# rmcar17/SpectralClusterSupertree

Measured on AMD Instinct MI355X. Metric: top-level PCG build + Fiedler solve wall-time (s) at N taxa, 1/2/4/8 MI355X, lower is better.
Workload: dtype f64 (loop operator: fp32 image of W; fp64 renewal + confirmation)

## Files before the change

include/scs_hip.h:

```cpp
#ifndef SCS_HIP_H
#define SCS_HIP_H

#include <stddef.h>
#include <stdint.h>

#ifdef __cplusplus
extern "C" {
#endif

#define SCS_OK 0
#define SCS_EINVAL (-1)
#define SCS_EHIP (-2)
#define SCS_ENOMEM (-3)
#define SCS_ECOMM (-4)
#define SCS_ENOCONV (-5)
#define SCS_EUNSUP (-6)

#define SCS_UNIQUE_ID_BYTES 128

typedef struct scs_ctx scs_ctx;
typedef struct scs_tables scs_tables;
typedef struct scs_graph scs_graph;

typedef struct scs_stats {
// ... 279 lines not shown
int scs_debug_update(scs_ctx *ctx, double *y, int32_t ldy, int32_t y_col0, int32_t kc, double alpha,
                     const double *a, int32_t lda, int32_t a_col0, int32_t ka, const double *c,
                     int32_t ldc, double sign, int32_t n);

int scs_debug_small_svqb(scs_ctx *ctx, const double *g, int32_t k, double drop_tol, double *t_out,
                         int32_t *mask_out);

int scs_debug_small_rr(scs_ctx *ctx, const double *tm, int32_t nparts, int32_t nq, int32_t b, const int32_t *mask,
                       double drop_tol, int32_t exact_from, int32_t start, double *c_out, double *d_out,
                       double *theta_out, int32_t *mask_p_out, int32_t *mask_out);

int scs_debug_small_orth(scs_ctx *ctx, const double *partial, int32_t nparts, int32_t b, double drop_tol,
                         const double *theta, int32_t layout, double *coef_out, int32_t *mask_out,
                         double *report_out);

#define SCS_DEBUG_PANEL_PAD 16
int scs_debug_panel(scs_ctx *ctx, int32_t which, int32_t b, int32_t n, const double *q, const double *aq,
                    const double *u, const double *coef_a, const double *coef_b, const double *theta,
                    const double *dinv, const double *ypart, int32_t nseg, int32_t blocks, double *q_out,
                    double *aq_out, double *partial_out, double *zt_out);

int scs_debug_comm_selftest(scs_ctx *ctx, int32_t count, const double *host_in, double *host_out);

int scs_debug_copy_bandwidth(scs_ctx *ctx, int64_t bytes, int32_t reps, double *gbs_out);

int scs_debug_scan(scs_ctx *ctx, int32_t op, int32_t n_parts, int64_t n, const int32_t *in, int32_t *out);

int scs_debug_graph_raw(scs_ctx *ctx, scs_graph *graph, int32_t what, void *out, int32_t *info_out);

int scs_debug_block_records(scs_ctx *ctx, const scs_tables *tables, int32_t t_begin, int32_t t_end, int32_t row_begin,
                            int32_t row_end, int32_t kind, int32_t *spos_out, double *gap_out, int32_t *argpos_out,
                            int32_t *depth_out, int32_t *cnt_out);

int scs_debug_split_plan(int32_t n_trees, const int64_t *node_off, int32_t *tpb_out, int32_t *n_groups_out,
                         uint8_t *staged_out);

int scs_debug_score_plan(const scs_tables *sources, int32_t n_trees, const int64_t *tree_off, int32_t super_leaves,
                         int32_t max_batch_trees, int64_t extra_per_leaf, int64_t extra_per_tree,
                         int32_t *n_batches_out, int32_t *bstart_out, int64_t *info_out, int32_t *words_out,
                         int32_t *zb_out, int64_t *wg_out);

int scs_debug_branch_plan(const scs_tables *sources, int32_t n_trees, const int64_t *tree_off, int32_t super_leaves,
                          int32_t max_batch_trees, int64_t extra_per_leaf, int64_t extra_per_tree,
                          int32_t max_lds_bytes, int32_t *n_batches_out, int32_t *bstart_out, int64_t *bt_out,
                          int64_t *tx_out, int64_t *call_out);

int scs_debug_placement_plan(const scs_tables *sources, int32_t n_trees, const int64_t *tree_off, int32_t super_leaves,
                             int32_t max_batch_trees, int32_t max_lds_bytes, int32_t n_queries,
                             int32_t n_sub_queries, int32_t n_degrees, const int32_t *degrees, int32_t *n_batches_out,
                             int32_t *bstart_out, int64_t *pl_out, int64_t *cp_out, int64_t *blk_out, int64_t *py_out);

int scs_debug_parsimony_plan(const scs_tables *sources, int32_t n_trees, const int64_t *tree_off, const int64_t *chars,
                             int32_t n_nodes, const int32_t *parent, int32_t max_batch_trees, int32_t max_pass_words,
                             int32_t *n_batches_out, int32_t *bstart_out, int64_t *info_out, int64_t *batch_out);

int scs_debug_source_pairs_plan(const scs_tables *sources, int32_t n_trees, const int64_t *tree_off, int32_t n_taxa,
                                int32_t n_rows, int32_t max_batch_trees, int32_t max_lds_bytes, int32_t *n_batches_out,
                                int32_t *bstart_out, int64_t *info_out, int64_t *tile_out);

int scs_debug_coverage_plan(const scs_tables *sources, int32_t n_trees, const int64_t *tree_off, int32_t n_taxa,
                            int32_t n_rows, int32_t min_trees, int32_t max_batch_rows, int32_t max_reg_words,
                            int32_t matrices_wanted, int64_t *info_out, int64_t *batches_out);

#ifdef __cplusplus
}
#endif
// ... 2 lines not shown
```

spectralclustersupertree_amd/_native.py:

```python

from __future__ import annotations

import ctypes as C
from pathlib import Path

import numpy as np

_PKG = Path(__file__).resolve().parent
LIB_PATH = _PKG / "libscs_hip.so"

UNIQUE_ID_BYTES = 128
BUILD_MONOTONE = 1
BUILD_SHARED = 2
BUILD_UPPER = 4
BUILD_SCATTER = 8


class ScsError(RuntimeError):

    def __init__(self, code: int, message: str) -> None:
        super().__init__(f"libscs_hip error {code}: {message}")
        self.code = code


# ... 145 lines not shown
    "scs_graph_download": (C.c_int, [_P, _P, _DP]),
    "scs_graph_download_rows": (C.c_int, [_P, _P, _I32, _I32, _DP]),
    "scs_graph_degrees": (C.c_int, [_P, _P, _DP]),
    "scs_graph_free": (C.c_int, [_P, _P]),
    "scs_fiedler": (C.c_int, [_P, _P, _DP, C.c_double, _I32, _I32, _DP, C.POINTER(Stats)]),
    "scs_small_solve": (C.c_int, [_P, _I32, _IP, _IP, _IP, _IP, _IP, _IP, _DP, _DP, _IP, _DP, _DP, _DP]),
    "scs_small_solve_begin": (C.c_int, [_P, _I32, _IP, _IP, _IP, _IP, _IP, _IP, _DP, _DP, _IP, _I32,
                                        C.POINTER(C.c_int32)]),
    "scs_small_solve_begin_forest": (C.c_int, [_P, _P, _IP, _I32, _I32, _IP, _I32, _P]),
    "scs_small_solve_end": (C.c_int, [_P, _I32, _DP, _DP, _DP]),
    "scs_debug_small_inputs": (C.c_int, [_P, _I32, _IP, _IP, _IP, _DP, _DP]),
    "scs_debug_tables_download": (C.c_int, [_P, _P, _LP, _IP, _IP, _DP, _DP, _LP]),
    "scs_debug_loop_policy": (C.c_int, [C.c_double, _I32, C.c_double, C.c_double, _I32, _I32, _DP, _IP]),
    "scs_debug_jacobi": (C.c_int, [_P, _DP, _I32, _DP, _DP]),
    "scs_debug_gram": (C.c_int, [_P, _DP, _DP, _I32, _I32, _I32, _I32, _DP]),
    "scs_debug_apply": (C.c_int, [_P, _P, _DP, _I32, _DP]),
    "scs_debug_apply_ex": (C.c_int, [_P, _P, _DP, _I32, _I32, _I32, _DP, _IP]),
    "scs_debug_team_apply": (C.c_int, [_P, _P, _DP, _DP, _I32, _I32, _I32, _I32, _DP, _DP, _DP, _LP]),
    "scs_debug_gram_ex": (C.c_int, [_P, _DP, _I32, _I32, _I32, _DP, _I32, _I32, _I32, _I32, _I32, _I32, _DP]),
    "scs_debug_update": (C.c_int, [_P, _DP, _I32, _I32, _I32, C.c_double, _DP, _I32, _I32, _I32, _DP, _I32,
                                   C.c_double, _I32]),
    "scs_debug_small_svqb": (C.c_int, [_P, _DP, _I32, C.c_double, _DP, _IP]),
    "scs_debug_small_rr": (C.c_int, [_P, _DP, _I32, _I32, _I32, _IP, C.c_double, _I32, _I32, _DP, _DP, _DP, _IP,
                                     _IP]),
    "scs_debug_small_orth": (C.c_int, [_P, _DP, _I32, _I32, C.c_double, _DP, _I32, _DP, _IP, _DP]),
    "scs_debug_panel": (C.c_int, [_P, _I32, _I32, _I32, _DP, _DP, _DP, _DP, _DP, _DP, _DP, _DP, _I32, _I32, _DP,
                                  _DP, _DP, _DP]),
    "scs_debug_comm_selftest": (C.c_int, [_P, _I32, _DP, _DP]),
    "scs_debug_copy_bandwidth": (C.c_int, [_P, C.c_int64, _I32, _DP]),
    "scs_debug_scan": (C.c_int, [_P, _I32, _I32, C.c_int64, _IP, _IP]),
    "scs_debug_split_plan": (C.c_int, [_I32, _LP, _P, _P, _P]),
    "scs_debug_graph_raw": (C.c_int, [_P, _P, _I32, _P, _IP]),
    "scs_debug_block_records": (C.c_int, [_P, _P, _I32, _I32, _I32, _I32, _I32, _IP, _DP, _IP, _IP, _IP]),
    "scs_debug_score_plan": (C.c_int, [_P, _I32, _LP, _I32, _I32, C.c_int64, C.c_int64, _P, _IP, _LP, _IP, _IP, _LP]),
    "scs_debug_branch_plan": (C.c_int, [_P, _I32, _LP, _I32, _I32, C.c_int64, C.c_int64, _I32, _P, _IP, _LP, _LP, _LP]),
    "scs_debug_placement_plan": (C.c_int, [_P, _I32, _LP, _I32, _I32, _I32, _I32, _I32, _I32, _IP, _IP, _IP, _LP, _LP,
                                           _LP, _LP]),
    "scs_debug_parsimony_plan": (C.c_int, [_P, _I32, _LP, _LP, _I32, _IP, _I32, _I32, _P, _IP, _LP, _LP]),
    "scs_debug_source_pairs_plan": (C.c_int, [_P, _I32, _LP, _I32, _I32, _I32, _I32, _P, _IP, _LP, _LP]),
    "scs_debug_coverage_plan": (C.c_int, [_P, _I32, _LP, _I32, _I32, _I32, _I32, _I32, _I32, _LP, _LP]),
}

_lib = None


def load_library() -> C.CDLL:
    global _lib
    if _lib is not None:
        return _lib
    if not LIB_PATH.exists():
        msg = (
            f"{LIB_PATH} not found: build it with `python -c 'import __graft_entry__ as g; g.build()'` "
            "or `make -C spectralclustersupertree_amd/csrc`.  There is no CPU fallback."
        )
        raise ImportError(msg)
    lib = C.CDLL(str(LIB_PATH))
    for name, (restype, argtypes) in SIGNATURES.items():
        fn = getattr(lib, name)
        fn.restype = restype
        fn.argtypes = argtypes
    have = int(lib.scs_version())
    if have != ABI_VERSION:
        msg = f"{LIB_PATH} reports ABI version {have}, this package binds {ABI_VERSION}: rebuild the library"
        raise ImportError(msg)
    _lib = lib
    return lib
# ... 48 lines not shown
```

spectralclustersupertree_amd/backend.py:

```python

from __future__ import annotations

import ctypes as C
import os

import numpy as np

from spectralclustersupertree_amd import _env
from spectralclustersupertree_amd import _native as nv
from spectralclustersupertree_amd.flatten import TreeTables

DEFAULT_TOL = 1e-13
DEFAULT_MAX_ITER = 2000

_M, _N, _Q, _QN, _QK = ("m",), ("n_nodes",), ("nq",), ("nq", "n_nodes"), ("nq", "top_k")


def _resident_solve() -> bool:
    return bool(int(_env.probe("SCS_RESIDENT_SOLVE", "1")))


class Device:

    def __init__(self, device: int = 0, rank: int = 0, world: int = 1, unique_id: bytes | None = None,
# ... 684 lines not shown
    out["py_bstart"] = bstart[2, : k + 1].astype(np.int64)
    rows = py.reshape(-1)[: k * len(deg) * 4].reshape(k, len(deg), 4)
    for i, key in enumerate(("words", "stride", "acc_lds", "lds")):
        out[f"py_{key}"] = rows[:, :, i].copy()
    return out


def debug_parsimony_plan(sources, parent, chars=None, batch_trees: int = 0, pass_words: int = 0) -> dict:
    handle, off = (sources._h, None) if isinstance(sources, DeviceTables) else (None, sources)
    if off is not None:
        off = np.ascontiguousarray(off, dtype=np.int64)
    m = sources.n_trees if off is None else len(off) - 1
    parent = np.ascontiguousarray(parent, dtype=np.int32)
    if chars is not None:
        chars = np.ascontiguousarray(chars, dtype=np.int64)
        if chars.shape != (m,):
            msg = f"chars must have one entry per source tree ({m}), not shape {chars.shape}"
            raise ValueError(msg)
    nb = C.c_int32(0)
    bstart = np.zeros(m + 1, dtype=np.int32)
    info = np.zeros(8, dtype=np.int64)
    rows = np.zeros((max(m, 1), 2), dtype=np.int64)
    nv.check(nv.load_library().scs_debug_parsimony_plan(
        handle, m, None if off is None else nv.lptr(off), None if chars is None else nv.lptr(chars), len(parent),
        nv.iptr(parent), int(batch_trees), int(pass_words), C.byref(nb), nv.iptr(bstart), nv.lptr(info),
        nv.lptr(rows)))
    k = int(nb.value)
    keys = ("pass_words", "frame_depth", "counter_bits", "lds_bytes", "frames_in_block", "extra_per_leaf",
            "extra_per_tree", "super_tips")
    return {"bstart": bstart[: k + 1].astype(np.int64), "passes": rows[:k, 0].copy(), "words": rows[:k, 1].copy(),
            **{key: int(info[i]) for i, key in enumerate(keys)}}


def debug_source_pairs_plan(sources, n_taxa: int = 0, n_rows: int | None = None, batch_trees: int = 0,
                            lds_bytes: int = 0) -> dict:
    handle, off = (sources._h, None) if isinstance(sources, DeviceTables) else (None, sources)
    if off is not None:
        off = np.ascontiguousarray(off, dtype=np.int64)
    m = sources.n_trees if off is None else len(off) - 1
    lib = nv.load_library()
    nb = C.c_int32(0)
    bstart = np.zeros(m + 1, dtype=np.int32)
    info = np.zeros(6, dtype=np.int64)
    args = (handle, m, None if off is None else nv.lptr(off), int(n_taxa), m if n_rows is None else int(n_rows),
            int(batch_trees), int(lds_bytes), C.byref(nb), nv.iptr(bstart), nv.lptr(info))
    nv.check(lib.scs_debug_source_pairs_plan(*args, None))
    k = int(nb.value)
    tiles = np.zeros((k, k, 7), dtype=np.int64)
    nv.check(lib.scs_debug_source_pairs_plan(*args, nv.lptr(tiles)))
    keys = ("levels", "row_stride", "slab_stride", "slab_wgs", "workspace", "lds_cap")
    return {"bstart": bstart[: k + 1].astype(np.int64), **{key: int(info[i]) for i, key in enumerate(keys)},
            "width": tiles[:, :, 0].copy(), "lds": tiles[:, :, 1].copy(), "slab": tiles[:, :, 2].copy(),
            "need": tiles[:, :, 3].copy(), "threads": tiles[:, :, 4].copy(), "grid_limit": tiles[:, :, 5].copy(),
            "rows_per_launch": tiles[:, :, 6].copy()}


def debug_coverage_plan(sources, n_taxa: int = 0, n_rows: int | None = None, min_trees: int = 1, batch_rows: int = 0,
                        reg_words: int = 0, matrices: int = 0) -> dict:
    handle, m = (sources._h, sources.n_trees) if isinstance(sources, DeviceTables) else (None, int(sources))
    lib = nv.load_library()
    info = np.zeros(12, dtype=np.int64)
    args = (handle, m, None, int(n_taxa), -1 if n_rows is None else int(n_rows), int(min_trees), int(batch_rows),
            int(reg_words), int(matrices), nv.lptr(info))
    nv.check(lib.scs_debug_coverage_plan(*args, None))
    batches = np.zeros((int(info[7]), 4), dtype=np.int64)
    nv.check(lib.scs_debug_coverage_plan(*args, nv.lptr(batches) if len(batches) else None))
# ... 151 lines not shown
        flags = nv.BUILD_MONOTONE if self.monotone else 0
        if upper:
            flags |= nv.BUILD_UPPER
            shared = False
        if scatter:
            flags |= nv.BUILD_SCATTER
            shared = False
        if shared is None:
            shared = self.dev.world > 1
        if shared:
            flags |= nv.BUILD_SHARED
        nv.check(self.dev._lib.scs_pcg_build(self.dev._ctx, self._h, row_begin, row_end, flags,
                                             C.byref(handle), C.byref(stats)))
        graph = DeviceGraph(self.dev, handle, stats.as_dict())
        graph.upper = bool(upper)
        return graph

    def block_records(self, kind: str, t_begin: int = 0, t_end: int | None = None, row_begin: int = 0,
                      row_end: int | None = None) -> dict:
        t_end = self.n_trees if t_end is None else t_end
        row_end = self.n_taxa if row_end is None else row_end
        code = {"mono": 0, "wide": 1, "general": 2}[kind]
        nb, nt = (max(row_end - row_begin, 0) + 63) // 64, max(t_end - t_begin, 0)
        spos = np.empty((nb, nt, 64), dtype=np.int32)
        gap = np.empty((nb, nt, 64), dtype=np.float64)
        argpos = np.empty((nb, nt, 64), dtype=np.int32)
        depth = np.empty((nb, nt, 64), dtype=np.int32) if code == 2 else None
        cnt = np.empty((nb, nt), dtype=np.int32)
        nv.check(self.dev._lib.scs_debug_block_records(
            self.dev._ctx, self._h, int(t_begin), int(t_end), int(row_begin), int(row_end), code, nv.iptr(spos),
            nv.dptr(gap), nv.iptr(argpos), nv.iptr(depth) if depth is not None else None, nv.iptr(cnt)))
        return {"spos": spos, "gap": gap, "argpos": argpos, "depth": depth, "cnt": cnt}


    def matrix_free_graph(self, max_block: int = 8) -> "DeviceGraph":
        handle = C.c_void_p()
        nv.check(self.dev._lib.scs_graph_matrix_free(self.dev._ctx, self._h, int(max_block), C.byref(handle)))
        return DeviceGraph(self.dev, handle, {})


class DeviceGraph:
    def __init__(self, dev: Device, handle, build_stats: dict | None = None) -> None:
        self.dev, self._h = dev, handle
        self.build_stats = build_stats or {}
        self.upper = False

    def free(self) -> None:
        if self._h:
            self.dev._lib.scs_graph_free(self.dev._ctx, self._h)
            self._h = C.c_void_p()

    def __del__(self) -> None:
        try:
            self.free()
        except Exception:
            pass

    @property
    def shape(self) -> tuple[int, int, int]:
        n, rb, re_ = C.c_int32(), C.c_int32(), C.c_int32()
        nv.check(self.dev._lib.scs_graph_shape(self._h, C.byref(n), C.byref(rb), C.byref(re_)))
        return n.value, rb.value, re_.value

    def contract(self, group_start: np.ndarray) -> "DeviceGraph":
        gs = np.ascontiguousarray(group_start, dtype=np.int32)
        handle = C.c_void_p()
# ... 109 lines not shown
```

spectralclustersupertree_amd/csrc/scs_build.hip:

```cpp

#include <algorithm>

#include "scs_internal.h"

typedef unsigned long long u64;
typedef unsigned int u32;

constexpr u32 DEPTH_INF = 0xFFFFFFFFu;


__device__ __forceinline__ void rmq_offsets(int m, int a, int b, int (&o)[2]) {
    const int k = 31 - __clz(b - a);
    o[0] = k * m + a;
    o[1] = k * m + b - (1 << k);
}

template <typename K>
__device__ __forceinline__ K rmq_min(const K *__restrict__ base, int m, int a, int b) {
    int o[2];
    rmq_offsets(m, a, b, o);
    const K x = base[o[0]], y = base[o[1]];
    return x < y ? x : y;
}

// ... 86 lines not shown
        const int half = 1 << (k - 1), last = m - (1 << k);
        const argmin_t *am_prev = am + (int64_t)(k - 2) * m;
        argmin_t *am_cur = am + (int64_t)(k - 1) * m;
        for (int p0 = threadIdx.x; p0 <= last; p0 += 1024 * FUSED_UNROLL) {
            K a[FUSED_UNROLL], b[FUSED_UNROLL];
            int oa[FUSED_UNROLL], ob[FUSED_UNROLL];
#pragma unroll
            for (int u = 0; u < FUSED_UNROLL; ++u) {
                const int p = p0 + u * 1024;
                oa[u] = ob[u] = 0;
                if (p <= last) {
                    a[u] = prev[p];
                    b[u] = prev[p + half];
                    if (k > 1) {
                        oa[u] = (int)am_prev[p];
                        ob[u] = (int)am_prev[p + half];
                    }
                }
            }
#pragma unroll
            for (int u = 0; u < FUSED_UNROLL; ++u) {
                const int p = p0 + u * 1024;
                if (p <= last) {
                    cur[p] = pick(a[u], b[u]);
                    am_cur[p] = (argmin_t)(pick.right_less(a[u], b[u]) ? half + ob[u] : oa[u]);
                }
            }
        }
        __syncthreads();
    }
}
constexpr int SPARSE_FUSED_MAX_LEAVES = 32768;
static_assert(SPARSE_FUSED_MAX_LEAVES <= (1 << ARGMIN_MAX_LEVEL), "every level of a fused table has an argmin level");
struct pick_smaller_value {
    __device__ double operator()(double a, double b) const { return a < b ? a : b; }
    __device__ bool right_less(double a, double b) const { return b < a; }
};

__device__ __forceinline__ double min_f64(double a, double b) {
#ifdef SCS_MIN_ASM
    double r;
    asm("v_min_f64 %0, %1, %2" : "=v"(r) : "v"(a), "v"(b));
    return r;
#else
    return __builtin_fmin(a, b);
#endif
}

#include "scs_mono.h"
#include "scs_mono_wide.h"
#include "scs_gen.h"
struct pick_shallower_pair {
    __device__ gap_entry operator()(const gap_entry a, const gap_entry b) const { return gap_min(a, b); }
    __device__ bool right_less(const gap_entry a, const gap_entry b) const { return b.d < a.d; }
};

__global__ __launch_bounds__(256) void k_scatter_atomic(const int64_t *__restrict__ tree_off,
                                                         const int32_t *__restrict__ leaf_taxon, int t0,
                                                         const int64_t *__restrict__ st_off,
                                                         const double *__restrict__ stv,
                                                         double *__restrict__ w, int64_t ld) {
    const int tl = blockIdx.y;
    const int64_t off = tree_off[t0 + tl];
    const int nl = (int)(tree_off[t0 + tl + 1] - off);
    const int m = nl - 1;
    const int nbk = (nl + 63) / 64;
// ... 387 lines not shown
__global__ void k_tile_lists(const int2 *__restrict__ tiles, int n_tiles, const unsigned char *__restrict__ rec,
                             int rec_bytes, int cnt_off, int n_batch, const unsigned char *__restrict__ pcol,
                             int32_t *__restrict__ lists, int32_t *__restrict__ list_cnt) {
    const int i = blockIdx.x * blockDim.x + threadIdx.x;
    if (i >= n_tiles) return;
    const int2 tile = tiles[i];
    const unsigned char *rb = rec + (int64_t)tile.x * n_batch * rec_bytes + cnt_off;
    const unsigned char *pc = pcol + (int64_t)tile.y * n_batch;
    int32_t *out = lists + (int64_t)i * n_batch;
    int c = 0;
    for (int t = 0; t < n_batch; ++t)
        if (pc[t] && *(const int *)(rb + (int64_t)t * rec_bytes) > 0) out[c++] = t;
    list_cnt[i] = c;
}

constexpr int PIPE_NG = 2;

namespace {

enum { PREP_MONO = 0, PREP_WIDE = 1, PREP_GEN = 2, PREP_NO_RECORDS = 3 };

struct prep_batch {
    const scs_tables *tb;
    int t0, nb;
    int kind;
    int32_t *pos;
    int64_t npad;
    const int64_t *st_off;
    const int64_t *am_off;
    void *st;
    argmin_t *am;
    unsigned char *rec;
    int n_blocks, row_begin, row_end;
};

int64_t table_entries(int64_t m) { return (int64_t)levels_for(m) * m; }
int64_t argmin_entries(int64_t m) { return (int64_t)argmin_levels(levels_for(m)) * m; }

int prep_piece(const prep_batch &b, int tl0, int np, hipStream_t s) {
    if (np <= 0) return SCS_OK;
    const scs_tables *tb = b.tb;
    int max_levels = 0;
    int64_t max_n = 0;
    for (int t = b.t0 + tl0; t < b.t0 + tl0 + np; ++t) {
        const int64_t nt = tb->h_tree_off[t + 1] - tb->h_tree_off[t];
        max_levels = std::max(max_levels, levels_for(nt - 1));
        max_n = std::max(max_n, nt);
    }
    const dim3 grid_l((unsigned)((max_n + 255) / 256), (unsigned)np);
    const dim3 grid_r((unsigned)b.n_blocks, (unsigned)np);
    const bool fused = max_n <= SPARSE_FUSED_MAX_LEAVES && max_levels > 1;
    if (b.kind != PREP_GEN) {
        double *st = (double *)b.st;
        k_positions_values<<<grid_l, 256, 0, s>>>(tb->d_tree_off, tb->d_leaf_taxon, tb->d_adj_depth, tb->d_adj_val,
                                                  tb->d_tree_w, b.t0, tl0, b.pos, b.npad, b.st_off, st);
        if (fused)
            k_sparse_levels_fused<double><<<(unsigned)np, 1024, 0, s>>>(tb->d_tree_off, b.t0, tl0, b.st_off, st, b.am_off,
                                                                        b.am, pick_smaller_value{});
        else
            for (int k = 1; k < max_levels; ++k)
                k_sparse_level<double><<<grid_l, 256, 0, s>>>(tb->d_tree_off, b.t0, tl0, k, b.st_off, st, b.am_off, b.am,
                                                              pick_smaller_value{});
        if (b.kind == PREP_WIDE)
            k_block_records_wide<PIPE_NG><<<grid_r, 64, 0, s>>>(tb->d_tree_off, b.t0, tl0, b.nb, b.pos, b.npad, b.st_off, st,
                                                          b.am_off, b.am, b.row_begin, b.row_end, b.rec);
        else if (b.kind == PREP_MONO)
            k_block_records_mono<<<grid_r, 64, 0, s>>>(tb->d_tree_off, b.t0, tl0, b.nb, b.pos, b.npad, b.st_off, st,
                                                       b.am_off, b.am, b.row_begin, b.row_end, b.rec);
    } else {
        gap_entry *st = (gap_entry *)b.st;
        k_positions_pairs<<<grid_l, 256, 0, s>>>(tb->d_tree_off, tb->d_leaf_taxon, tb->d_adj_depth, tb->d_adj_val,
                                                 tb->d_tree_w, b.t0, tl0, b.pos, b.npad, b.st_off, st);
        if (fused)
            k_sparse_levels_fused<gap_entry><<<(unsigned)np, 1024, 0, s>>>(tb->d_tree_off, b.t0, tl0, b.st_off, st,
                                                                           b.am_off, b.am, pick_shallower_pair{});
        else
            for (int k = 1; k < max_levels; ++k)
                k_sparse_level<gap_entry><<<grid_l, 256, 0, s>>>(tb->d_tree_off, b.t0, tl0, k, b.st_off, st, b.am_off,
                                                                 b.am, pick_shallower_pair{});
        k_block_records_gen<<<grid_r, 64, 0, s>>>(tb->d_tree_off, b.t0, tl0, b.nb, b.pos, b.npad, b.st_off, st, b.am_off,
                                                  b.am, b.row_begin, b.row_end, b.rec);
    }
    SCS_HIP_CHECK(hipGetLastError());
    return SCS_OK;
}

struct pinned_ref {
    scs_ctx *ctx;
    hipStream_t stream;
    void *p = nullptr;
    bool in_flight = false;
    pinned_ref(scs_ctx *c, hipStream_t s) : ctx(c), stream(s) {}
    ~pinned_ref() {
        if (!p) return;
        if (in_flight) hipStreamSynchronize(stream);
        scs_pinned_release(ctx, p);
    }
};

}

extern "C" int scs_pcg_build(scs_ctx *ctx, const scs_tables *tb, int32_t row_begin,
                             int32_t row_end, int32_t flags, scs_graph **out,
                             scs_build_stats *stats) {
    SCS_REQUIRE(ctx && tb && out, "scs_pcg_build: null argument");
    SCS_REQUIRE((flags & ~(SCS_BUILD_MONOTONE | SCS_BUILD_SHARED | SCS_BUILD_UPPER | SCS_BUILD_SCATTER)) == 0,
// ... 250 lines not shown
        const size_t need_pos = (size_t)nb * npad * 4;
        const size_t need_st = (size_t)h_st_off[nb] * entry_bytes + 64;
        const size_t need_am = (size_t)h_am_off[nb] * sizeof(argmin_t) + 64;
        const size_t need_rec = (size_t)n_blocks * nb * rec_bytes;
        const int wide_min_trees = wide_forced ? 1 : 96;
        const bool wide_b = wide && (nb >= wide_min_trees || (groups.size() >= 8 * 256 && nb >= 16));
        if (wide_b) {
            ++spec_batches;
            spec_trees += nb;
            single_batch_spec = true;
        }
        SCS_TRY(d_pos.alloc(need_pos));
        SCS_TRY(d_st.alloc(need_st));
        SCS_TRY(d_am.alloc(need_am));
        SCS_TRY(d_rec.alloc(need_rec));

        SCS_HIP_CHECK(hipEventRecord(ev_prep.a, s));
        SCS_HIP_CHECK(hipMemsetAsync(d_pos.p, 0xFF, need_pos, s));
        prep_batch pb;
        pb.tb = tb;
        pb.t0 = t0;
        pb.nb = nb;
        pb.kind = !monotone ? PREP_GEN : wide_b ? PREP_WIDE : scatter ? PREP_NO_RECORDS : PREP_MONO;
        pb.pos = (int32_t *)d_pos.p;
        pb.npad = npad;
        pb.st_off = (const int64_t *)d_stoff.p + off_at[bi];
        pb.am_off = pb.st_off + nb + 1;
        pb.st = d_st.p;
        pb.am = (argmin_t *)d_am.p;
        pb.rec = (unsigned char *)d_rec.p;
        pb.n_blocks = n_blocks;
        pb.row_begin = b_row_begin;
        pb.row_end = b_row_end;
        for (int p0 = t0; p0 < t1;) {
            int p1 = t1;
            if (by_arrival)
                for (const int32_t c : tb->late_start)
                    if (c > p0 && c < p1) p1 = c;
            SCS_TRY(scs_tables_wait(ctx, tb, p1, s));
            SCS_TRY(prep_piece(pb, p0 - t0, p1 - p0, s));
            ++prep_pieces;
            p0 = p1;
        }
        SCS_HIP_CHECK(hipEventRecord(ev_prep.b, s));

        SCS_HIP_CHECK(hipEventRecord(ev_acc.a, s));
        const unsigned nt = (unsigned)tiles.size();
        if (scatter) {
            const int64_t nbk = (max_n + 63) / 64;
            k_scatter_atomic<<<dim3((unsigned)(nbk * (nbk + 1) / 2), (unsigned)nb), 256, 0, s>>>(
                tb->d_tree_off, tb->d_leaf_taxon, t0, pb.st_off, (const double *)d_st.p,
                g->d_w, g->ld);
        } else if (monotone) {
            mono_params mp;
            mp.tiles = (const int2 *)d_tiles.p;
            mp.rec = (const unsigned char *)d_rec.p;
            mp.pos = (const int32_t *)d_pos.p;
            mp.npad = npad;
            mp.stv = (const double *)d_st.p;
            mp.n_batch = nb;
            mp.w = w_base;
            mp.ld = g->ld;
            mp.n = n;
            mp.row_begin = b_row_begin;
            mp.row_end = b_row_end;
            mp.load_w = bi > 0;
// ... 474 lines not shown
            return SCS_EUNSUP;
        }
        if (!img_rows && !(g->row_begin == 0 && rows == g->n)) {
            scs_set_error("scs_debug_graph_raw: a row block [%d, %d) of %d on one rank has no image", g->row_begin,
                          g->row_end, g->n);
            return SCS_EUNSUP;
        }
    }
    info_out[0] = rows;
    info_out[1] = (int32_t)g->ld;
    info_out[2] = g->col0;
    info_out[3] = (what == 1 && img_rows) ? 1 : 0;
    if (!out) return SCS_OK;
    SCS_HIP_CHECK(hipSetDevice(ctx->device));
    if (what == 1) {
        SCS_TRY(scs_graph_prepare_degrees_begin(ctx, g, true));
        SCS_TRY(scs_graph_prepare_degrees(ctx, g));
        if (!g->have_w32 || !g->d_w32) {
            scs_set_error("scs_debug_graph_raw: the image could not be made (no memory)");
            return SCS_EUNSUP;
        }
    }
    if (what == 2) SCS_TRY(scs_graph_prepare_degrees(ctx, g));
    SCS_HIP_CHECK(hipStreamSynchronize(ctx->stream));
    if (what == 2)
        SCS_HIP_CHECK(hipMemcpy(out, g->d_deg, (size_t)g->n * 8, hipMemcpyDeviceToHost));
    else if (what == 1)
        SCS_HIP_CHECK(hipMemcpy(out, g->d_w32, (size_t)rows * (size_t)g->ld * 4, hipMemcpyDeviceToHost));
    else
        SCS_HIP_CHECK(hipMemcpy(out, g->d_w, (size_t)rows * (size_t)g->ld * 8, hipMemcpyDeviceToHost));
    return SCS_OK;
}

extern "C" int scs_debug_block_records(scs_ctx *ctx, const scs_tables *tb, int32_t t_begin, int32_t t_end,
                                       int32_t row_begin, int32_t row_end, int32_t kind, int32_t *spos_out,
                                       double *gap_out, int32_t *argpos_out, int32_t *depth_out, int32_t *cnt_out) {
    SCS_REQUIRE(ctx && tb && spos_out && gap_out && argpos_out && cnt_out, "scs_debug_block_records: null argument");
    SCS_REQUIRE(kind == PREP_MONO || kind == PREP_WIDE || kind == PREP_GEN,
                "scs_debug_block_records: kind must be 0 (mono), 1 (wide) or 2 (general), not %d", kind);
    SCS_REQUIRE(t_begin >= 0 && t_begin < t_end && t_end <= tb->n_trees,
                "scs_debug_block_records: bad tree range [%d, %d) of %d", t_begin, t_end, tb->n_trees);
    SCS_REQUIRE(row_begin >= 0 && row_begin < row_end && row_end <= tb->n_taxa,
                "scs_debug_block_records: bad row range [%d, %d) for %d taxa", row_begin, row_end, tb->n_taxa);
    SCS_HIP_CHECK(hipSetDevice(ctx->device));
    hipStream_t s = ctx->stream;
    const int n = tb->n_taxa, nb = t_end - t_begin;
    const int n_blocks = (row_end - row_begin + SCS_TR - 1) / SCS_TR;
    const int n_cgroups = (n + MONO_TCW - 1) / MONO_TCW;
    const int64_t npad = scs_round_up((int64_t)n_cgroups * MONO_TCW, SCS_NPAD);
    const size_t entry_bytes = kind == PREP_GEN ? sizeof(gap_entry) : 8;
    const size_t rec_bytes = kind == PREP_GEN ? G3_BYTES : kind == PREP_WIDE ? wide_layout<PIPE_NG>::BYTES : R3_BYTES;
    std::vector<int64_t> off(2 * (size_t)(nb + 1), 0);
    int64_t *st_off = off.data(), *am_off = off.data() + nb + 1;
    for (int t = 0; t < nb; ++t) {
        const int64_t m = tb->h_tree_off[t_begin + t + 1] - tb->h_tree_off[t_begin + t] - 1;
        st_off[t + 1] = st_off[t] + table_entries(m);
        am_off[t + 1] = am_off[t] + argmin_entries(m);
    }
    dev_buf d_pos(ctx), d_st(ctx), d_am(ctx), d_off(ctx), d_rec(ctx);
    const size_t need_pos = (size_t)nb * npad * 4, need_rec = (size_t)n_blocks * nb * rec_bytes;
    SCS_TRY(d_pos.alloc(need_pos));
    SCS_TRY(d_st.alloc((size_t)st_off[nb] * entry_bytes + 64));
    SCS_TRY(d_am.alloc((size_t)am_off[nb] * sizeof(argmin_t) + 64));
    SCS_TRY(d_off.alloc(off.size() * 8));
    SCS_TRY(d_rec.alloc(need_rec));
    SCS_HIP_CHECK(hipMemcpy(d_off.p, off.data(), off.size() * 8, hipMemcpyHostToDevice));
    SCS_HIP_CHECK(hipMemsetAsync(d_pos.p, 0xFF, need_pos, s));
    prep_batch pb;
    pb.tb = tb;
    pb.t0 = t_begin;
    pb.nb = nb;
    pb.kind = kind;
    pb.pos = (int32_t *)d_pos.p;
    pb.npad = npad;
    pb.st_off = (const int64_t *)d_off.p;
    pb.am_off = pb.st_off + nb + 1;
    pb.st = d_st.p;
    pb.am = (argmin_t *)d_am.p;
    pb.rec = (unsigned char *)d_rec.p;
    pb.n_blocks = n_blocks;
    pb.row_begin = row_begin;
    pb.row_end = row_end;
    SCS_TRY(scs_tables_wait(ctx, tb, t_end, s));
    SCS_TRY(prep_piece(pb, 0, nb, s));
    std::vector<unsigned char> rec(need_rec);
    SCS_HIP_CHECK(hipMemcpyAsync(rec.data(), d_rec.p, need_rec, hipMemcpyDeviceToHost, s));
    SCS_HIP_CHECK(hipStreamSynchronize(s));
    const int o_spos = kind == PREP_GEN ? G3_SPOS : kind == PREP_WIDE ? wide_layout<PIPE_NG>::SPOS : R3_SPOS;
    const int o_gap = kind == PREP_GEN ? G3_GV : kind == PREP_WIDE ? wide_layout<PIPE_NG>::G : R3_G;
    const int o_arg = kind == PREP_GEN ? G3_ARGPOS : kind == PREP_WIDE ? wide_layout<PIPE_NG>::ARGPOS : R3_ARGPOS;
    const int o_cnt = kind == PREP_GEN ? G3_CNT : kind == PREP_WIDE ? wide_layout<PIPE_NG>::CNT : R3_CNT;
    for (size_t i = 0; i < (size_t)n_blocks * nb; ++i) {
        const unsigned char *r = rec.data() + i * rec_bytes;
        memcpy(spos_out + i * 64, r + o_spos, 256);
        memcpy(gap_out + i * 64, r + o_gap, 512);
        memcpy(argpos_out + i * 64, r + o_arg, 256);
        if (kind == PREP_GEN && depth_out) memcpy(depth_out + i * 64, r + G3_GD, 256);
        memcpy(cnt_out + i, r + o_cnt, 4);
    }
    return SCS_OK;
}
```

Before: 0.01391.

## Build sparse-table levels in LDS with multi-block split per tree

Adds a kernel that builds the range-minimum sparse-table levels and argmin tables inside LDS, reading each level from shared memory rather than global memory. Writes to global memory are split across several blocks per tree so more CUs take part when trees are few. It is selected when a tree's leaves fit in LDS and exceed a size gate; otherwise the fused or per-level kernels run as before. Each block recomputes every level redundantly, and new debug entry points are added for inspection.

```diff
diff --git a/include/scs_hip.h b/include/scs_hip.h
--- a/include/scs_hip.h
+++ b/include/scs_hip.h
@@ -335,6 +335,15 @@
                             int32_t row_end, int32_t kind, int32_t *spos_out, double *gap_out, int32_t *argpos_out,
                             int32_t *depth_out, int32_t *cnt_out);
 
+int scs_debug_level_tables(scs_ctx *ctx, const scs_tables *tables, int32_t t_begin, int32_t t_end, int32_t pairs,
+                           int32_t parts, int32_t lds, void *st_out, uint16_t *am_out, int64_t *info_out);
+
+int scs_debug_record_seeds(scs_ctx *ctx, const scs_tables *tables, int32_t t_begin, int32_t t_end, int32_t row_begin,
+                           int32_t row_end, int32_t kind, double *seed_out, uint32_t *depth_out);
+
+int scs_debug_levels_path(int64_t max_leaves, int32_t entry_bytes, int32_t trees, int32_t lds_bytes, int32_t n_cu,
+                          int32_t gated, int32_t *kind_out, int32_t *parts_out);
+
 int scs_debug_split_plan(int32_t n_trees, const int64_t *node_off, int32_t *tpb_out, int32_t *n_groups_out,
                          uint8_t *staged_out);
 
diff --git a/spectralclustersupertree_amd/_native.py b/spectralclustersupertree_amd/_native.py
--- a/spectralclustersupertree_amd/_native.py
+++ b/spectralclustersupertree_amd/_native.py
@@ -201,6 +201,9 @@
     "scs_debug_split_plan": (C.c_int, [_I32, _LP, _P, _P, _P]),
     "scs_debug_graph_raw": (C.c_int, [_P, _P, _I32, _P, _IP]),
     "scs_debug_block_records": (C.c_int, [_P, _P, _I32, _I32, _I32, _I32, _I32, _IP, _DP, _IP, _IP, _IP]),
+    "scs_debug_level_tables": (C.c_int, [_P, _P, _I32, _I32, _I32, _I32, _I32, _P, _P, _LP]),
+    "scs_debug_record_seeds": (C.c_int, [_P, _P, _I32, _I32, _I32, _I32, _I32, _DP, _IP]),
+    "scs_debug_levels_path": (C.c_int, [C.c_int64, _I32, _I32, _I32, _I32, _I32, _IP, _IP]),
     "scs_debug_score_plan": (C.c_int, [_P, _I32, _LP, _I32, _I32, C.c_int64, C.c_int64, _P, _IP, _LP, _IP, _IP, _LP]),
     "scs_debug_branch_plan": (C.c_int, [_P, _I32, _LP, _I32, _I32, C.c_int64, C.c_int64, _I32, _P, _IP, _LP, _LP, _LP]),
     "scs_debug_placement_plan": (C.c_int, [_P, _I32, _LP, _I32, _I32, _I32, _I32, _I32, _I32, _IP, _IP, _IP, _LP, _LP,
diff --git a/spectralclustersupertree_amd/backend.py b/spectralclustersupertree_amd/backend.py
--- a/spectralclustersupertree_amd/backend.py
+++ b/spectralclustersupertree_amd/backend.py
@@ -740,6 +740,14 @@
             **{key: int(info[i]) for i, key in enumerate(keys)}}
 
 
+def debug_levels_path(max_leaves: int, entry_bytes: int, trees: int, lds_bytes: int, n_cu: int,
+                      gated: bool = True) -> tuple[int, int]:
+    kind, parts = C.c_int32(-1), C.c_int32(-1)
+    nv.check(nv.load_library().scs_debug_levels_path(int(max_leaves), int(entry_bytes), int(trees), int(lds_bytes),
+                                                     int(n_cu), int(bool(gated)), C.byref(kind), C.byref(parts)))
+    return int(kind.value), int(parts.value)
+
+
 def debug_source_pairs_plan(sources, n_taxa: int = 0, n_rows: int | None = None, batch_trees: int = 0,
                             lds_bytes: int = 0) -> dict:
     handle, off = (sources._h, None) if isinstance(sources, DeviceTables) else (None, sources)
@@ -957,6 +965,31 @@
             nv.dptr(gap), nv.iptr(argpos), nv.iptr(depth) if depth is not None else None, nv.iptr(cnt)))
         return {"spos": spos, "gap": gap, "argpos": argpos, "depth": depth, "cnt": cnt}
 
+    def record_seeds(self, kind: str, t_begin: int = 0, t_end: int | None = None, row_begin: int = 0,
+                     row_end: int | None = None) -> dict:
+        t_end = self.n_trees if t_end is None else t_end
+        row_end = self.n_taxa if row_end is None else row_end
+        code = {"mono": 0, "wide": 1, "general": 2}[kind]
+        segs = 7 if code == 1 else 3
+        nb, nt = (max(row_end - row_begin, 0) + 63) // 64, max(t_end - t_begin, 0)
+        seed = np.empty((nb, nt, segs, 64), dtype=np.float64)
+        depth = np.empty((nb, nt, segs, 64), dtype=np.uint32) if code == 2 else None
+        nv.check(self.dev._lib.scs_debug_record_seeds(
+            self.dev._ctx, self._h, int(t_begin), int(t_end), int(row_begin), int(row_end), code, nv.dptr(seed),
+            depth.ctypes.data if depth is not None else None))
+        return {"seed": seed, "depth": depth}
+
+    def level_tables(self, t_begin: int = 0, t_end: int | None = None, pairs: bool = False, parts: int = 0,
+                     lds: int = 1) -> dict:
+        t_end = self.n_trees if t_end is None else t_end
+        info = np.zeros(6, dtype=np.int64)
+        args = (self.dev._ctx, self._h, int(t_begin), int(t_end), int(bool(pairs)), int(parts), int(lds))
+        nv.check(self.dev._lib.scs_debug_level_tables(*args, None, None, nv.lptr(info)))
+        st = np.empty((int(info[0]), 4), dtype=np.uint32) if pairs else np.empty(int(info[0]), dtype=np.float64)
+        am = np.empty(int(info[1]), dtype=np.uint16)
+        nv.check(self.dev._lib.scs_debug_level_tables(*args, st.ctypes.data, am.ctypes.data, nv.lptr(info)))
+        return {"st": st, "am": am, "kernel": int(info[2]), "parts": int(info[3]), "lds_bytes": int(info[4]),
+                "n_cu": int(info[5])}
 
     def matrix_free_graph(self, max_block: int = 8) -> "DeviceGraph":
         handle = C.c_void_p()
diff --git a/spectralclustersupertree_amd/csrc/scs_build.hip b/spectralclustersupertree_amd/csrc/scs_build.hip
--- a/spectralclustersupertree_amd/csrc/scs_build.hip
+++ b/spectralclustersupertree_amd/csrc/scs_build.hip
@@ -142,6 +142,64 @@
 }
 constexpr int SPARSE_FUSED_MAX_LEAVES = 32768;
 static_assert(SPARSE_FUSED_MAX_LEAVES <= (1 << ARGMIN_MAX_LEVEL), "every level of a fused table has an argmin level");
+
+constexpr int LEVELS_LDS_MAX_PARTS = 8;
+constexpr int LEVELS_LDS_PER_VALUE = 16, LEVELS_LDS_PER_PAIR = 10;
+template <typename K, typename PICK, int PER>
+__global__ __launch_bounds__(1024) void k_sparse_levels_lds(const int64_t *__restrict__ tree_off, int t0, int tl0,
+                                                             int parts, const int64_t *__restrict__ st_off,
+                                                             K *__restrict__ st, const int64_t *__restrict__ am_off,
+                                                             argmin_t *__restrict__ am_all, PICK pick) {
+    extern __shared__ __attribute__((aligned(16))) unsigned char s_levels[];
+    const int tl = tl0 + (int)blockIdx.x / parts, part = (int)blockIdx.x % parts;
+    const int m = (int)(tree_off[t0 + tl + 1] - tree_off[t0 + tl]) - 1;
+    if (m < 2 || m > 1024 * PER) return;
+    K *lev = (K *)s_levels;
+    argmin_t *la = (argmin_t *)(s_levels + (size_t)m * sizeof(K));
+    K *base = st + st_off[tl];
+    argmin_t *am = am_all + am_off[tl];
+    const int tid = threadIdx.x;
+    const int slice = ((m + 63) / 64 + parts - 1) / parts * 64;
+    const int lo = min(m, part * slice), hi = part == parts - 1 ? m : min(m, (part + 1) * slice);
+    for (int p = tid; p < m; p += 1024) lev[p] = base[p];
+    __syncthreads();
+    for (int k = 1; (1 << k) <= m; ++k) {
+        const int half = 1 << (k - 1), last = m - (1 << k);
+        K r[PER];
+        argmin_t o[PER];
+#pragma unroll
+        for (int u = 0; u < PER; ++u) {
+            const int p = tid + u * 1024;
+            if (p <= last) {
+                const K a = lev[p], b = lev[p + half];
+                int oa = 0, ob = 0;
+                if (k > 1) {
+                    oa = (int)la[p];
+                    ob = (int)la[p + half];
+                }
+                r[u] = pick(a, b);
+                o[u] = (argmin_t)(pick.right_less(a, b) ? half + ob : oa);
+            }
+        }
+        __syncthreads();
+        K *cur = base + (int64_t)k * m;
+        argmin_t *am_cur = am + (int64_t)(k - 1) * m;
+#pragma unroll
+        for (int u = 0; u < PER; ++u) {
+            const int p = tid + u * 1024;
+            if (p <= last) {
+                lev[p] = r[u];
+                la[p] = o[u];
+                if (p >= lo && p < hi) {
+                    cur[p] = r[u];
+                    am_cur[p] = o[u];
+                }
+            }
+        }
+        __syncthreads();
+    }
+}
+
 struct pick_smaller_value {
     __device__ double operator()(double a, double b) const { return a < b ? a : b; }
     __device__ bool right_less(double a, double b) const { return b < a; }
@@ -595,12 +653,44 @@
     argmin_t *am;
     unsigned char *rec;
     int n_blocks, row_begin, row_end;
+    int lds_bytes = 0, n_cu = 0;
+    int levels_lds = -1;
+    int levels_parts = 0;
 };
+
+enum { LEVELS_PER_LEVEL = 0, LEVELS_FUSED = 1, LEVELS_LDS = 2 };
+struct levels_path {
+    int kind, parts;
+};
+constexpr int LEVELS_LDS_MIN_LEAVES = 3072;
+levels_path levels_path_of(int64_t max_leaves, int entry_bytes, int trees, int lds_bytes, int n_cu, bool gated) {
+    const int64_t m = max_leaves - 1;
+    levels_path lp = {LEVELS_PER_LEVEL, 1};
+    if (m < 2 || max_leaves > SPARSE_FUSED_MAX_LEAVES) return lp;
+    lp.kind = LEVELS_FUSED;
+    if (gated && max_leaves < LEVELS_LDS_MIN_LEAVES) return lp;
+    const int per = entry_bytes == 8 ? LEVELS_LDS_PER_VALUE : LEVELS_LDS_PER_PAIR;
+    if (m * (entry_bytes + (int64_t)sizeof(argmin_t)) <= (int64_t)lds_bytes && m <= 1024 * (int64_t)per) {
+        lp.kind = LEVELS_LDS;
+        lp.parts = std::min(std::max(n_cu / std::max(trees, 1), 1), LEVELS_LDS_MAX_PARTS);
+    }
+    return lp;
+}
+
+template <typename K, typename PICK, int PER>
+int launch_levels_lds(const prep_batch &b, int tl0, int np, int parts, int64_t max_m, PICK pick, hipStream_t s) {
+    const size_t lds = (size_t)max_m * (sizeof(K) + sizeof(argmin_t));
+    SCS_HIP_CHECK(hipFuncSetAttribute((const void *)k_sparse_levels_lds<K, PICK, PER>,
+                                      hipFuncAttributeMaxDynamicSharedMemorySize, (int)lds));
+    k_sparse_levels_lds<K, PICK, PER><<<(unsigned)np * (unsigned)parts, 1024, lds, s>>>(
+        b.tb->d_tree_off, b.t0, tl0, parts, b.st_off, (K *)b.st, b.am_off, b.am, pick);
+    return SCS_OK;
+}
 
 int64_t table_entries(int64_t m) { return (int64_t)levels_for(m) * m; }
 int64_t argmin_entries(int64_t m) { return (int64_t)argmin_levels(levels_for(m)) * m; }
 
-int prep_piece(const prep_batch &b, int tl0, int np, hipStream_t s) {
+int prep_piece(const prep_batch &b, int tl0, int np, hipStream_t s, levels_path *taken = nullptr) {
     if (np <= 0) return SCS_OK;
     const scs_tables *tb = b.tb;
     int max_levels = 0;
@@ -612,12 +702,27 @@
     }
     const dim3 grid_l((unsigned)((max_n + 255) / 256), (unsigned)np);
     const dim3 grid_r((unsigned)b.n_blocks, (unsigned)np);
-    const bool fused = max_n <= SPARSE_FUSED_MAX_LEAVES && max_levels > 1;
+    const int entry_bytes = b.kind == PREP_GEN ? (int)sizeof(gap_entry) : 8;
+    int lds_mode = b.levels_lds < 0 ? 1 : b.levels_lds;
+    if (b.levels_lds < 0)
+        if (const char *e = scs_dbg("SCS_LEVELS_LDS")) lds_mode = atoi(e);
+    levels_path lp = levels_path_of(max_n, entry_bytes, np, lds_mode != 0 ? b.lds_bytes : 0, b.n_cu, lds_mode != 2);
+    if (lp.kind == LEVELS_LDS) {
+        int forced = b.levels_parts;
+        if (forced <= 0)
+            if (const char *e = scs_dbg("SCS_LEVELS_PARTS")) forced = atoi(e);
+        if (forced > 0) lp.parts = std::min(forced, LEVELS_LDS_MAX_PARTS);
+    }
+    if (taken) *taken = lp;
+    const bool fused = lp.kind == LEVELS_FUSED;
     if (b.kind != PREP_GEN) {
         double *st = (double *)b.st;
         k_positions_values<<<grid_l, 256, 0, s>>>(tb->d_tree_off, tb->d_leaf_taxon, tb->d_adj_depth, tb->d_adj_val,
                                                   tb->d_tree_w, b.t0, tl0, b.pos, b.npad, b.st_off, st);
-        if (fused)
+        if (lp.kind == LEVELS_LDS)
+            SCS_TRY((launch_levels_lds<double, pick_smaller_value, LEVELS_LDS_PER_VALUE>(b, tl0, np, lp.parts, max_n - 1,
+                                                                                         pick_smaller_value{}, s)));
+        else if (fused)
             k_sparse_levels_fused<double><<<(unsigned)np, 1024, 0, s>>>(tb->d_tree_off, b.t0, tl0, b.st_off, st, b.am_off,
                                                                         b.am, pick_smaller_value{});
         else
@@ -634,7 +739,10 @@
         gap_entry *st = (gap_entry *)b.st;
         k_positions_pairs<<<grid_l, 256, 0, s>>>(tb->d_tree_off, tb->d_leaf_taxon, tb->d_adj_depth, tb->d_adj_val,
                                                  tb->d_tree_w, b.t0, tl0, b.pos, b.npad, b.st_off, st);
-        if (fused)
+        if (lp.kind == LEVELS_LDS)
+            SCS_TRY((launch_levels_lds<gap_entry, pick_shallower_pair, LEVELS_LDS_PER_PAIR>(b, tl0, np, lp.parts, max_n - 1,
+                                                                                            pick_shallower_pair{}, s)));
+        else if (fused)
             k_sparse_levels_fused<gap_entry><<<(unsigned)np, 1024, 0, s>>>(tb->d_tree_off, b.t0, tl0, b.st_off, st,
                                                                            b.am_off, b.am, pick_shallower_pair{});
         else
@@ -951,6 +1059,8 @@
         pb.n_blocks = n_blocks;
         pb.row_begin = b_row_begin;
         pb.row_end = b_row_end;
+        pb.lds_bytes = ctx->max_lds_bytes;
+        pb.n_cu = ctx->n_cu;
         for (int p0 = t0; p0 < t1;) {
             int p1 = t1;
             if (by_arrival)
@@ -1491,6 +1601,74 @@
     return SCS_OK;
 }
 
+namespace {
+
+struct debug_prep {
+    int nb = 0, n_blocks = 0;
+    size_t entry_bytes = 0, rec_bytes = 0, need_rec = 0;
+    std::vector<int64_t> off;
+    dev_buf d_pos, d_st, d_am, d_off, d_rec;
+    levels_path taken = {LEVELS_PER_LEVEL, 1};
+    explicit debug_prep(scs_ctx *ctx) : d_pos(ctx), d_st(ctx), d_am(ctx), d_off(ctx), d_rec(ctx) {}
+    const int64_t *st_off() const { return off.data(); }
+    const int64_t *am_off() const { return off.data() + nb + 1; }
+    int run(scs_ctx *ctx, const scs_tables *tb, int32_t t_begin, int32_t t_end, int32_t row_begin, int32_t row_end,
+            int kind, int levels_lds, int levels_parts) {
+        SCS_HIP_CHECK(hipSetDevice(ctx->device));
+        hipStream_t s = ctx->stream;
+        const int n = tb->n_taxa;
+        nb = t_end - t_begin;
+        n_blocks = (row_end - row_begin + SCS_TR - 1) / SCS_TR;
+        const int n_cgroups = (n + MONO_TCW - 1) / MONO_TCW;
+        const int64_t npad = scs_round_up((int64_t)n_cgroups * MONO_TCW, SCS_NPAD);
+        entry_bytes = kind == PREP_GEN ? sizeof(gap_entry) : 8;
+        rec_bytes = kind == PREP_GEN ? G3_BYTES : kind == PREP_WIDE ? wide_layout<PIPE_NG>::BYTES : R3_BYTES;
+        off.assign(2 * (size_t)(nb + 1), 0);
+        int64_t *so = off.data(), *ao = off.data() + nb + 1;
+        for (int t = 0; t < nb; ++t) {
+            const int64_t m = tb->h_tree_off[t_begin + t + 1] - tb->h_tree_off[t_begin + t] - 1;
+            so[t + 1] = so[t] + table_entries(m);
+            ao[t + 1] = ao[t] + argmin_entries(m);
+        }
+        const size_t need_pos = (size_t)nb * npad * 4;
+        const size_t need_st = (size_t)so[nb] * entry_bytes + 64, need_am = (size_t)ao[nb] * sizeof(argmin_t) + 64;
+        need_rec = (size_t)n_blocks * nb * rec_bytes;
+        SCS_TRY(d_pos.alloc(need_pos));
+        SCS_TRY(d_st.alloc(need_st));
+        SCS_TRY(d_am.alloc(need_am));
+        SCS_TRY(d_off.alloc(off.size() * 8));
+        SCS_TRY(d_rec.alloc(need_rec));
+        SCS_HIP_CHECK(hipMemcpy(d_off.p, off.data(), off.size() * 8, hipMemcpyHostToDevice));
+        SCS_HIP_CHECK(hipMemsetAsync(d_pos.p, 0xFF, need_pos, s));
+        SCS_HIP_CHECK(hipMemsetAsync(d_st.p, 0, need_st, s));
+        SCS_HIP_CHECK(hipMemsetAsync(d_am.p, 0, need_am, s));
+        prep_batch pb;
+        pb.tb = tb;
+        pb.t0 = t_begin;
+        pb.nb = nb;
+        pb.kind = kind;
+        pb.pos = (int32_t *)d_pos.p;
+        pb.npad = npad;
+        pb.st_off = (const int64_t *)d_off.p;
+        pb.am_off = pb.st_off + nb + 1;
+        pb.st = d_st.p;
+        pb.am = (argmin_t *)d_am.p;
+        pb.rec = (unsigned char *)d_rec.p;
+        pb.n_blocks = n_blocks;
+        pb.row_begin = row_begin;
+        pb.row_end = row_end;
+        pb.lds_bytes = ctx->max_lds_bytes;
+        pb.n_cu = ctx->n_cu;
+        pb.levels_lds = levels_lds;
+        pb.levels_parts = levels_parts;
+        SCS_TRY(scs_tables_wait(ctx, tb, t_end, s));
+        SCS_TRY(prep_piece(pb, 0, nb, s, &taken));
+        return SCS_OK;
+    }
+};
+
+}
+
 extern "C" int scs_debug_block_records(scs_ctx *ctx, const scs_tables *tb, int32_t t_begin, int32_t t_end,
                                        int32_t row_begin, int32_t row_end, int32_t kind, int32_t *spos_out,
                                        double *gap_out, int32_t *argpos_out, int32_t *depth_out, int32_t *cnt_out) {
@@ -1501,55 +1679,17 @@
                 "scs_debug_block_records: bad tree range [%d, %d) of %d", t_begin, t_end, tb->n_trees);
     SCS_REQUIRE(row_begin >= 0 && row_begin < row_end && row_end <= tb->n_taxa,
                 "scs_debug_block_records: bad row range [%d, %d) for %d taxa", row_begin, row_end, tb->n_taxa);
-    SCS_HIP_CHECK(hipSetDevice(ctx->device));
-    hipStream_t s = ctx->stream;
-    const int n = tb->n_taxa, nb = t_end - t_begin;
-    const int n_blocks = (row_end - row_begin + SCS_TR - 1) / SCS_TR;
-    const int n_cgroups = (n + MONO_TCW - 1) / MONO_TCW;
-    const int64_t npad = scs_round_up((int64_t)n_cgroups * MONO_TCW, SCS_NPAD);
-    const size_t entry_bytes = kind == PREP_GEN ? sizeof(gap_entry) : 8;
-    const size_t rec_bytes = kind == PREP_GEN ? G3_BYTES : kind == PREP_WIDE ? wide_layout<PIPE_NG>::BYTES : R3_BYTES;
-    std::vector<int64_t> off(2 * (size_t)(nb + 1), 0);
-    int64_t *st_off = off.data(), *am_off = off.data() + nb + 1;
-    for (int t = 0; t < nb; ++t) {
-        const int64_t m = tb->h_tree_off[t_begin + t + 1] - tb->h_tree_off[t_begin + t] - 1;
-        st_off[t + 1] = st_off[t] + table_entries(m);
-        am_off[t + 1] = am_off[t] + argmin_entries(m);
-    }
-    dev_buf d_pos(ctx), d_st(ctx), d_am(ctx), d_off(ctx), d_rec(ctx);
-    const size_t need_pos = (size_t)nb * npad * 4, need_rec = (size_t)n_blocks * nb * rec_bytes;
-    SCS_TRY(d_pos.alloc(need_pos));
-    SCS_TRY(d_st.alloc((size_t)st_off[nb] * entry_bytes + 64));
-    SCS_TRY(d_am.alloc((size_t)am_off[nb] * sizeof(argmin_t) + 64));
-    SCS_TRY(d_off.alloc(off.size() * 8));
-    SCS_TRY(d_rec.alloc(need_rec));
-    SCS_HIP_CHECK(hipMemcpy(d_off.p, off.data(), off.size() * 8, hipMemcpyHostToDevice));
-    SCS_HIP_CHECK(hipMemsetAsync(d_pos.p, 0xFF, need_pos, s));
-    prep_batch pb;
-    pb.tb = tb;
-    pb.t0 = t_begin;
-    pb.nb = nb;
-    pb.kind = kind;
-    pb.pos = (int32_t *)d_pos.p;
-    pb.npad = npad;
-    pb.st_off = (const int64_t *)d_off.p;
-    pb.am_off = pb.st_off + nb + 1;
-    pb.st = d_st.p;
-    pb.am = (argmin_t *)d_am.p;
-    pb.rec = (unsigned char *)d_rec.p;
-    pb.n_blocks = n_blocks;
-    pb.row_begin = row_begin;
-    pb.row_end = row_end;
-    SCS_TRY(scs_tables_wait(ctx, tb, t_end, s));
-    SCS_TRY(prep_piece(pb, 0, nb, s));
-    std::vector<unsigned char> rec(need_rec);
-    SCS_HIP_CHECK(hipMemcpyAsync(rec.data(), d_rec.p, need_rec, hipMemcpyDeviceToHost, s));
-    SCS_HIP_CHECK(hipStreamSynchronize(s));
+    debug_prep dp(ctx);
+    SCS_TRY(dp.run(ctx, tb, t_begin, t_end, row_begin, row_end, kind, -1, 0));
+    const size_t rec_bytes = dp.rec_bytes;
+    std::vector<unsigned char> rec(dp.need_rec);
+    SCS_HIP_CHECK(hipMemcpyAsync(rec.data(), dp.d_rec.p, dp.need_rec, hipMemcpyDeviceToHost, ctx->stream));
+    SCS_HIP_CHECK(hipStreamSynchronize(ctx->stream));
     const int o_spos = kind == PREP_GEN ? G3_SPOS : kind == PREP_WIDE ? wide_layout<PIPE_NG>::SPOS : R3_SPOS;
     const int o_gap = kind == PREP_GEN ? G3_GV : kind == PREP_WIDE ? wide_layout<PIPE_NG>::G : R3_G;
     const int o_arg = kind == PREP_GEN ? G3_ARGPOS : kind == PREP_WIDE ? wide_layout<PIPE_NG>::ARGPOS : R3_ARGPOS;
     const int o_cnt = kind == PREP_GEN ? G3_CNT : kind == PREP_WIDE ? wide_layout<PIPE_NG>::CNT : R3_CNT;
-    for (size_t i = 0; i < (size_t)n_blocks * nb; ++i) {
+    for (size_t i = 0; i < (size_t)dp.n_blocks * dp.nb; ++i) {
         const unsigned char *r = rec.data() + i * rec_bytes;
         memcpy(spos_out + i * 64, r + o_spos, 256);
         memcpy(gap_out + i * 64, r + o_gap, 512);
@@ -1559,3 +1699,81 @@
     }
     return SCS_OK;
 }
+
+extern "C" int scs_debug_record_seeds(scs_ctx *ctx, const scs_tables *tb, int32_t t_begin, int32_t t_end,
+                                      int32_t row_begin, int32_t row_end, int32_t kind, double *seed_out,
+                                      uint32_t *depth_out) {
+    const char *const who = "scs_debug_record_seeds";
+    SCS_REQUIRE(ctx && tb && seed_out, "%s: null argument", who);
+    SCS_REQUIRE(kind == PREP_MONO || kind == PREP_WIDE || kind == PREP_GEN,
+                "%s: kind must be 0 (mono), 1 (wide) or 2 (general), not %d", who, kind);
+    SCS_REQUIRE(t_begin >= 0 && t_begin < t_end && t_end <= tb->n_trees, "%s: bad tree range [%d, %d) of %d", who,
+                t_begin, t_end, tb->n_trees);
+    SCS_REQUIRE(row_begin >= 0 && row_begin < row_end && row_end <= tb->n_taxa,
+                "%s: bad row range [%d, %d) for %d taxa", who, row_begin, row_end, tb->n_taxa);
+    debug_prep dp(ctx);
+    SCS_TRY(dp.run(ctx, tb, t_begin, t_end, row_begin, row_end, kind, -1, 0));
+    std::vector<unsigned char> rec(dp.need_rec);
+    SCS_HIP_CHECK(hipMemcpyAsync(rec.data(), dp.d_rec.p, dp.need_rec, hipMemcpyDeviceToHost, ctx->stream));
+    SCS_HIP_CHECK(hipStreamSynchronize(ctx->stream));
+    const int segs = (kind == PREP_WIDE ? wide_layout<PIPE_NG>::NSEG : MONO_WAVES) - 1;
+    const int o_seed = kind == PREP_GEN ? G3_SEEDV : kind == PREP_WIDE ? wide_layout<PIPE_NG>::SEED : R3_SEED;
+    for (size_t i = 0; i < (size_t)dp.n_blocks * dp.nb; ++i) {
+        const unsigned char *r = rec.data() + i * dp.rec_bytes;
+        memcpy(seed_out + i * segs * 64, r + o_seed, (size_t)segs * 512);
+        if (kind == PREP_GEN && depth_out) memcpy(depth_out + i * segs * 64, r + G3_SEEDD, (size_t)segs * 256);
+    }
+    return SCS_OK;
+}
+
+extern "C" int scs_debug_level_tables(scs_ctx *ctx, const scs_tables *tb, int32_t t_begin, int32_t t_end,
+                                      int32_t pairs, int32_t parts, int32_t lds, void *st_out, uint16_t *am_out,
+                                      int64_t *info_out) {
+    const char *const who = "scs_debug_level_tables";
+    SCS_REQUIRE(ctx && tb && info_out, "%s: null argument", who);
+    SCS_REQUIRE((st_out == nullptr) == (am_out == nullptr), "%s: st_out and am_out go together", who);
+    SCS_REQUIRE(t_begin >= 0 && t_begin < t_end && t_end <= tb->n_trees, "%s: bad tree range [%d, %d) of %d", who,
+                t_begin, t_end, tb->n_trees);
+    SCS_REQUIRE(parts >= 0 && parts <= LEVELS_LDS_MAX_PARTS, "%s: parts = %d is not in [0, %d]", who, parts,
+                LEVELS_LDS_MAX_PARTS);
+    SCS_REQUIRE((pairs == 0 || pairs == 1) && lds >= 0 && lds <= 2, "%s: pairs is 0 or 1, lds 0, 1 or 2", who);
+    info_out[4] = ctx->max_lds_bytes;
+    info_out[5] = ctx->n_cu;
+    if (!st_out) {
+        int64_t st = 0, am = 0;
+        for (int t = t_begin; t < t_end; ++t) {
+            const int64_t m = tb->h_tree_off[t + 1] - tb->h_tree_off[t] - 1;
+            st += table_entries(m);
+            am += argmin_entries(m);
+        }
+        info_out[0] = st;
+        info_out[1] = am;
+        return SCS_OK;
+    }
+    debug_prep dp(ctx);
+    SCS_TRY(dp.run(ctx, tb, t_begin, t_end, 0, std::min<int32_t>(tb->n_taxa, SCS_TR), pairs ? PREP_GEN : PREP_NO_RECORDS,
+                   lds, parts));
+    info_out[0] = dp.st_off()[dp.nb];
+    info_out[1] = dp.am_off()[dp.nb];
+    info_out[2] = dp.taken.kind;
+    info_out[3] = dp.taken.parts;
+    SCS_HIP_CHECK(hipMemcpyAsync(st_out, dp.d_st.p, (size_t)info_out[0] * dp.entry_bytes, hipMemcpyDeviceToHost,
+                                 ctx->stream));
+    SCS_HIP_CHECK(hipMemcpyAsync(am_out, dp.d_am.p, (size_t)info_out[1] * sizeof(argmin_t), hipMemcpyDeviceToHost,
+                                 ctx->stream));
+    SCS_HIP_CHECK(hipStreamSynchronize(ctx->stream));
+    return SCS_OK;
+}
+
+extern "C" int scs_debug_levels_path(int64_t max_leaves, int32_t entry_bytes, int32_t trees, int32_t lds_bytes,
+                                     int32_t n_cu, int32_t gated, int32_t *kind_out, int32_t *parts_out) {
+    const char *const who = "scs_debug_levels_path";
+    SCS_REQUIRE(kind_out && parts_out, "%s: null argument", who);
+    SCS_REQUIRE(max_leaves >= 0 && trees >= 1 && lds_bytes >= 0 && n_cu >= 1, "%s: bad argument", who);
+    SCS_REQUIRE(entry_bytes == 8 || entry_bytes == (int32_t)sizeof(gap_entry), "%s: entry_bytes is 8 or %d, not %d", who,
+                (int)sizeof(gap_entry), entry_bytes);
+    const levels_path lp = levels_path_of(max_leaves, entry_bytes, trees, lds_bytes, n_cu, gated != 0);
+    *kind_out = lp.kind;
+    *parts_out = lp.parts;
+    return SCS_OK;
+}
```

Result: faster. 0.01374 (median of 6 runs) (-1.2%).
